# qiaozhijian/VCR-Net

Measured on NVIDIA B200. Metric: pairs/sec @1024 pts, higher is better.
Workload: dtype f16x3-split+f32acc (fp32-equivalent)

## Files before the change

### vcr_net_b200/csrc/knn.cu

```cuda
#include <atomic>
#include "tc_common.cuh"

namespace {

constexpr int TQ = 32;
constexpr int TC = 512;
constexpr int NT = 256;
constexpr int RPL = TC / 32;

template <bool TOKEN_MAJOR>
__global__ void knn_sqnorm_kernel(const float* __restrict__ x, int D, int N, float* __restrict__ xx) {
    const int b = blockIdx.y;
    const int i = blockIdx.x * blockDim.x + threadIdx.x;
    if (i >= N) return;
    const float* xb = x + (size_t)b * D * N;
    float acc = 0.f;
    for (int d = 0; d < D; ++d) {
        const float v = TOKEN_MAJOR ? xb[(size_t)i * D + d] : xb[(size_t)d * N + i];
        acc = fmaf(v, v, acc);
    }
    xx[(size_t)b * N + i] = acc;
}

__device__ __forceinline__ uint32_t okey(float v) {
    const uint32_t b = __float_as_uint(v + 0.f);
    return b ^ (uint32_t)(((int32_t)b >> 31) | 0x80000000);
}
__device__ __forceinline__ float okey_inv(uint32_t k) {
    return __uint_as_float((k & 0x80000000u) ? (k ^ 0x80000000u) : ~k);
}
struct Key { uint32_t hi, lo; };
__device__ __forceinline__ Key key_xchg(Key v, int j, bool take_max) {
    Key o;
    o.hi = __shfl_xor_sync(0xffffffffu, v.hi, j);
    o.lo = __shfl_xor_sync(0xffffffffu, v.lo, j);
    const bool gt = v.hi > o.hi || (v.hi == o.hi && v.lo > o.lo);
    return gt == take_max ? v : o;
}
__device__ __forceinline__ Key key_max(Key a, Key b) {
    return (a.hi > b.hi || (a.hi == b.hi && a.lo > b.lo)) ? a : b;
}

template <int W>
__device__ __forceinline__ void sort32_desc(Key (&v)[W], int lane) {
#pragma unroll
    for (int ks = 2; ks <= 32; ks <<= 1) {
#pragma unroll
        for (int j = ks >> 1; j > 0; j >>= 1) {
            const bool take_max = ((lane & j) == 0) == ((lane & ks) == 0);
#pragma unroll
            for (int w = 0; w < W; ++w) v[w] = key_xchg(v[w], j, take_max);
        }
    }
}
template <int W>
__device__ __forceinline__ void sort32_desc_f(float (&v)[W], int lane) {
#pragma unroll
    for (int ks = 2; ks <= 32; ks <<= 1) {
#pragma unroll
        for (int j = ks >> 1; j > 0; j >>= 1) {
            const bool take_max = ((lane & j) == 0) == ((lane & ks) == 0);
#pragma unroll
            for (int w = 0; w < W; ++w) {
                const float o = __shfl_xor_sync(0xffffffffu, v[w], j);
                v[w] = take_max ? fmaxf(v[w], o) : fminf(v[w], o);
            }
        }
    }
}
template <int W>
__device__ __forceinline__ void merge32_desc(Key (&run)[W], const Key (&add)[W], int lane) {
#pragma unroll
    for (int w = 0; w < W; ++w) {
        Key o;
        o.hi = __shfl_sync(0xffffffffu, add[w].hi, 31 - lane);
        o.lo = __shfl_sync(0xffffffffu, add[w].lo, 31 - lane);
        run[w] = key_max(run[w], o);
    }
#pragma unroll
    for (int j = 16; j > 0; j >>= 1) {
        const bool take_max = (lane & j) == 0;
#pragma unroll
        for (int w = 0; w < W; ++w) run[w] = key_xchg(run[w], j, take_max);
    }
}

template <int W, int TCN, int LDD, int CAP>
__device__ __forceinline__ bool filter_merge_t(const float* drows, const float (&tau)[W], Key (&run)[W], uint2* buf,
                                               int j0, int lane) {
    constexpr int RP = TCN / 32;
    const uint32_t lt = (1u << lane) - 1u;
    int cnt[W], off[W];
    int base = 0;
    __syncwarp();
#pragma unroll
    for (int w = 0; w < W; ++w) {
        const float* dr = drows + w * LDD + lane;
        float v[RP];
#pragma unroll
        for (int r = 0; r < RP; ++r) v[r] = dr[r * 32];
        off[w] = base;
        int n = base;
#pragma unroll
        for (int r = 0; r < RP; ++r) {
            const bool p = v[r] >= tau[w];
            const uint32_t bal = __ballot_sync(0xffffffffu, p);
            const int pos = n + __popc(bal & lt);
            if (p && pos < CAP) buf[pos] = make_uint2(~(uint32_t)(j0 + r * 32 + lane), okey(v[r]));
            n += __popc(bal);
        }
        cnt[w] = n - base;
        base = n;
    }
    __syncwarp();
    if (base > CAP) return false;
    int rounds = 0;
#pragma unroll
    for (int w = 0; w < W; ++w) rounds = max(rounds, (cnt[w] + 31) >> 5);
    for (int r = 0; r < rounds; ++r) {
        Key e[W];
#pragma unroll
        for (int w = 0; w < W; ++w) {
            const int p = r * 32 + lane;
            const uint2 t = p < cnt[w] ? buf[off[w] + p] : make_uint2(0u, 0u);
            e[w].lo = t.x; e[w].hi = t.y;
        }
        sort32_desc<W>(e, lane);
        merge32_desc<W>(run, e, lane);
    }
    return true;
}
template <int W>
__device__ __forceinline__ bool filter_merge(const float* drows, const float (&tau)[W], Key (&run)[W], uint2* buf,
                                             int j0, int lane) {
    return filter_merge_t<W, TC, TC, TC>(drows, tau, run, buf, j0, lane);
}

__device__ __forceinline__ void select_chunk(const float* dist, uint2* surv, Key (&run)[TQ / (NT / 32)], int j0, int kk,
                                             int warp, int lane, bool first) {
    constexpr int QWn = TQ / (NT / 32);
    uint2* buf = surv + (size_t)warp * TC;
    const float* drows = dist + (size_t)(warp * QWn) * TC;
    float tau[QWn];
    if (first) {
        float m[QWn];
#pragma unroll
        for (int w = 0; w < QWn; ++w) {
            const float* dr = drows + w * TC + lane;
            float mm = dr[0];
#pragma unroll
            for (int r = 1; r < RPL; ++r) mm = fmaxf(mm, dr[r * 32]);
            m[w] = mm;
        }
        sort32_desc_f<QWn>(m, lane);
#pragma unroll
        for (int w = 0; w < QWn; ++w) tau[w] = __shfl_sync(0xffffffffu, m[w], kk);
    } else {
#pragma unroll
        for (int w = 0; w < QWn; ++w) tau[w] = okey_inv(__shfl_sync(0xffffffffu, run[w].hi, kk));
    }
    if (!filter_merge<QWn>(drows, tau, run, buf, j0, lane)) {
#pragma unroll
        for (int w = 0; w < QWn; ++w) {
            float t1[1] = {tau[w]};
            Key r1[1] = {run[w]};
            filter_merge<1>(drows + w * TC, t1, r1, buf, j0, lane);
            run[w] = r1[0];
        }
    }
}

__device__ __forceinline__ void cp_async16(float* dst, const float* src, bool valid) {
    const uint32_t d = (uint32_t)__cvta_generic_to_shared(dst);
    const int sz = valid ? 16 : 0;
    asm volatile("cp.async.ca.shared.global [%0], [%1], 16, %2;\n" ::"r"(d), "l"(src), "r"(sz) : "memory");
}
__device__ __forceinline__ void cp_async_wait_all() { asm volatile("cp.async.wait_all;\n" ::: "memory"); }
__device__ __forceinline__ void cp_async_commit() { asm volatile("cp.async.commit_group;\n" ::: "memory"); }
template <int NPEND>
__device__ __forceinline__ void cp_async_wait_group() { asm volatile("cp.async.wait_group %0;\n" ::"n"(NPEND) : "memory"); }

template <int DCH, int DCP>
__device__ __forceinline__ void issue_slab(const float* __restrict__ xb, int D, int N, int j0, int q0, int d0,
                                           float* Cb, float* Qb, int tid) {
    constexpr int PPR = DCH / 4;
    constexpr int RPP = 256 / PPR;
    const int part = tid % PPR, r0 = tid / PPR;
    const bool dok = d0 + 4 * part < D;
    const float* src = xb + (size_t)(j0 + r0) * D + d0 + 4 * part;
    float* dst = Cb + r0 * DCP + 4 * part;
#pragma unroll
    for (int n = 0; n < 512 / RPP; ++n) {
        const bool ok = dok && j0 + r0 + n * RPP < N;
        cp_async16(dst + n * RPP * DCP, ok ? src + (size_t)n * RPP * D : xb, ok);
    }
    if (r0 < 32) {
        const bool ok = dok && q0 + r0 < N;
        cp_async16(Qb + r0 * DCP + 4 * part, ok ? xb + (size_t)(q0 + r0) * D + d0 + 4 * part : xb, ok);
    }
    cp_async_commit();
}

constexpr int QW = TQ / (NT / 32);
constexpr size_t SURV_BYTES = (size_t)(NT / 32) * TC * sizeof(uint2);

template <int DCH>
struct Smem {
    static constexpr int DCP = DCH == 4 ? 12 : DCH + 4;
    static constexpr size_t stage_bytes = (size_t)(TC + TQ) * DCP * sizeof(float);
    static constexpr size_t region0 = stage_bytes > SURV_BYTES ? stage_bytes : SURV_BYTES;
    static constexpr size_t total = region0 + (size_t)TC * sizeof(float) + (size_t)TQ * TC * sizeof(float);
};

template <int DCH, bool TOKEN_MAJOR>
__global__ void __launch_bounds__(NT, 2)
knn_select_kernel(const float* __restrict__ x, const float* __restrict__ xx, int D, int N, int k,
                  int32_t* __restrict__ idx32, int64_t* __restrict__ idx64, const int* __restrict__ redo) {
    if (redo != nullptr && redo[blockIdx.y * gridDim.x + blockIdx.x] == 0) return;
    using S = Smem<DCH>;
    constexpr int DCP = S::DCP;
    extern __shared__ __align__(16) unsigned char smem_raw[];
    float* Cs = reinterpret_cast<float*>(smem_raw);
    float* Qs = Cs + TC * DCP;
    uint2* surv = reinterpret_cast<uint2*>(smem_raw);
    float* xxc = reinterpret_cast<float*>(smem_raw + S::region0);
    float* dist = xxc + TC;

    const int tid = threadIdx.x, lane = tid & 31, warp = tid >> 5;
    const int qg = warp & 3, cg = warp >> 2;
    const int b = blockIdx.y, q0 = blockIdx.x * TQ;
    const float* xb = x + (size_t)b * D * N;
    const float* xxb = xx + (size_t)b * N;
    const bool vec = TOKEN_MAJOR && (D % 4 == 0) && ((reinterpret_cast<uintptr_t>(x) & 15) == 0);

    Key run[QW];
#pragma unroll
    for (int w = 0; w < QW; ++w) run[w].hi = run[w].lo = 0u;

    for (int j0 = 0; j0 < N; j0 += TC) {
        float acc[8][8];
#pragma unroll
        for (int qi = 0; qi < 8; ++qi)
#pragma unroll
            for (int ci = 0; ci < 8; ++ci) acc[qi][ci] = 0.f;

        const int nslab = (D + DCH - 1) / DCH;
        __syncthreads();
        if (vec) issue_slab<DCH, DCP>(xb, D, N, j0, q0, 0, Cs, Qs, tid);
        for (int c = tid; c < TC; c += NT) xxc[c] = (j0 + c < N) ? xxb[j0 + c] : 0.f;
        for (int si = 0; si < nslab; ++si) {
            const int d0 = si * DCH;
            const float* Cb = (vec && (si & 1)) ? dist : Cs;
            const float* Qb = Cb + TC * DCP;
            if (vec) {
                if (si + 1 < nslab) {
                    float* Cn = (si & 1) ? Cs : dist;
                    issue_slab<DCH, DCP>(xb, D, N, j0, q0, d0 + DCH, Cn, Cn + TC * DCP, tid);
                    cp_async_wait_group<1>();
                } else {
                    cp_async_wait_group<0>();
                }
            } else {
                for (int e = tid; e < (TC + TQ) * DCH; e += NT) {
                    int row, d;
                    if (TOKEN_MAJOR) { row = e / DCH; d = e - row * DCH; }
                    else if (e < TC * DCH) { d = e / TC; row = e - d * TC; }
                    else { const int e2 = e - TC * DCH; d = e2 / TQ; row = TC + e2 - d * TQ; }
                    const int g = row < TC ? j0 + row : q0 + (row - TC);
                    float v = 0.f;
                    if (g < N && d0 + d < D)
                        v = TOKEN_MAJOR ? xb[(size_t)g * D + d0 + d] : xb[(size_t)(d0 + d) * N + g];
                    Cs[row * DCP + d] = v;
                }
            }
            __syncthreads();

            const float* qrow = Qb + (qg * 8) * DCP;
            const float* crow = Cb + (cg * 256 + lane) * DCP;
            if (j0 + cg * 256 < N) {
#pragma unroll 1
            for (int d4 = 0; d4 < DCH / 4; ++d4) {
#pragma unroll
                for (int h = 0; h < 2; ++h) {
                    float4 cv[4];
#pragma unroll
                    for (int ci = 0; ci < 4; ++ci)
                        cv[ci] = *reinterpret_cast<const float4*>(crow + ((h * 4 + ci) * 32) * DCP + d4 * 4);
#pragma unroll
                    for (int qi = 0; qi < 8; ++qi) {
                        const float4 qv = *reinterpret_cast<const float4*>(qrow + qi * DCP + d4 * 4);
#pragma unroll
                        for (int ci = 0; ci < 4; ++ci) acc[qi][h * 4 + ci] = fmaf(qv.x, cv[ci].x, acc[qi][h * 4 + ci]);
#pragma unroll
                        for (int ci = 0; ci < 4; ++ci) acc[qi][h * 4 + ci] = fmaf(qv.y, cv[ci].y, acc[qi][h * 4 + ci]);
#pragma unroll
                        for (int ci = 0; ci < 4; ++ci) acc[qi][h * 4 + ci] = fmaf(qv.z, cv[ci].z, acc[qi][h * 4 + ci]);
#pragma unroll
                        for (int ci = 0; ci < 4; ++ci) acc[qi][h * 4 + ci] = fmaf(qv.w, cv[ci].w, acc[qi][h * 4 + ci]);
                    }
                }
            }
            }
            __syncthreads();
        }

        float xxq[8];
#pragma unroll
        for (int qi = 0; qi < 8; ++qi) {
            const int q = q0 + qg * 8 + qi;
            xxq[qi] = q < N ? xxb[q] : 0.f;
        }
#pragma unroll
        for (int ci = 0; ci < 8; ++ci) {
            const int c = cg * 256 + ci * 32 + lane;
            const float nxc = -xxc[c];
            const bool cvalid = j0 + c < N;
#pragma unroll
            for (int qi = 0; qi < 8; ++qi) {
                const float pd = __fsub_rn(__fsub_rn(nxc, -2.f * acc[qi][ci]), xxq[qi]);
                dist[(qg * 8 + qi) * TC + c] = cvalid ? pd : -INFINITY;
            }
        }
        __syncthreads();

        select_chunk(dist, surv, run, j0, k, warp, lane, j0 == 0);
    }

#pragma unroll
    for (int w = 0; w < QW; ++w) {
        const int q = q0 + warp * QW + w;
        if (q < N && lane >= 1 && lane <= k) {
            const int j = (int)(~run[w].lo);
            const size_t o = ((size_t)b * N + q) * k + lane - 1;
            if (idx32) idx32[o] = j;
            if (idx64) idx64[o] = (int64_t)j;
        }
    }
}

template <int DCH, bool TM>
int launch_knn(const float* x, const float* xx, int B, int D, int N, int k, int32_t* i32, int64_t* i64,
               cudaStream_t st, const int* redo = nullptr) {
    auto kern = knn_select_kernel<DCH, TM>;
    const size_t smem = Smem<DCH>::total;
    if (cudaFuncSetAttribute(kern, cudaFuncAttributeMaxDynamicSharedMemorySize, (int)smem) != cudaSuccess) return VCR_ERR_LAUNCH;
    dim3 grid(vcr_cdiv(N, TQ), B);
    kern<<<grid, NT, smem, st>>>(x, xx, D, N, k, i32, i64, redo);
    VCR_CHECK_LAUNCH();
    return VCR_OK;
}

template <int W, class F>
__device__ __forceinline__ bool filter_merge_fn(F&& get, const float (&tau)[W], Key (&run)[W], uint2* buf, int j0, int lane) {
    constexpr int RP = TC / 32;
    const uint32_t lt = (1u << lane) - 1u;
    int cnt[W], off[W];
    int base = 0;
    __syncwarp();
#pragma unroll
    for (int w = 0; w < W; ++w) {
        off[w] = base;
        int n = base;
#pragma unroll
        for (int r = 0; r < RP; ++r) {
            const float v = get(w, r);
            const bool p = v >= tau[w];
            const uint32_t bal = __ballot_sync(0xffffffffu, p);
            const int pos = n + __popc(bal & lt);
            if (p && pos < TC) buf[pos] = make_uint2(~(uint32_t)(j0 + r * 32 + lane), okey(v));
            n += __popc(bal);
        }
        cnt[w] = n - base;
        base = n;
    }
    __syncwarp();
    if (base > TC) return false;
    int rounds = 0;
#pragma unroll
    for (int w = 0; w < W; ++w) rounds = max(rounds, (cnt[w] + 31) >> 5);
    for (int r = 0; r < rounds; ++r) {
        Key e[W];
#pragma unroll
        for (int w = 0; w < W; ++w) {
            const int p = r * 32 + lane;
            const uint2 t = p < cnt[w] ? buf[off[w] + p] : make_uint2(0u, 0u);
            e[w].lo = t.x; e[w].hi = t.y;
        }
        sort32_desc<W>(e, lane);
        merge32_desc<W>(run, e, lane);
    }
    return true;
}

constexpr int QW3 = 2;
constexpr int TQ3 = QW3 * (NT / 32);
template <bool TOKEN_MAJOR>
__global__ void __launch_bounds__(NT, 4)
knn3_kernel(const float* __restrict__ x, const float* __restrict__ xx, int N, int k,
            int32_t* __restrict__ idx32, int64_t* __restrict__ idx64) {
    __shared__ float cs[4][TC];
    __shared__ uint2 surv[NT / 32][TC];
    const int tid = threadIdx.x, lane = tid & 31, warp = tid >> 5;
    const int b = blockIdx.y, q0 = blockIdx.x * TQ3;
    const float* xb = x + (size_t)b * 3 * N;
    const float* xxb = xx + (size_t)b * N;

    float qx[QW3], qy[QW3], qz[QW3], xxq[QW3];
#pragma unroll
    for (int w = 0; w < QW3; ++w) {
        const int q = min(q0 + warp * QW3 + w, N - 1);
        qx[w] = TOKEN_MAJOR ? xb[(size_t)q * 3 + 0] : xb[q];
        qy[w] = TOKEN_MAJOR ? xb[(size_t)q * 3 + 1] : xb[(size_t)N + q];
        qz[w] = TOKEN_MAJOR ? xb[(size_t)q * 3 + 2] : xb[2 * (size_t)N + q];
        xxq[w] = xxb[q];
    }
    Key run[QW3];
#pragma unroll
    for (int w = 0; w < QW3; ++w) run[w].hi = run[w].lo = 0u;
    uint2* buf = surv[warp];

    for (int j0 = 0; j0 < N; j0 += TC) {
        __syncthreads();
        for (int c = tid; c < TC; c += NT) {
            const int g = j0 + c;
            const bool ok = g < N;
            cs[0][c] = ok ? (TOKEN_MAJOR ? xb[(size_t)g * 3 + 0] : xb[g]) : 0.f;
            cs[1][c] = ok ? (TOKEN_MAJOR ? xb[(size_t)g * 3 + 1] : xb[(size_t)N + g]) : 0.f;
            cs[2][c] = ok ? (TOKEN_MAJOR ? xb[(size_t)g * 3 + 2] : xb[2 * (size_t)N + g]) : 0.f;
            cs[3][c] = ok ? xxb[g] : 0.f;
        }
        __syncthreads();
        auto pd = [&](int w, int r) -> float {
            const int c = r * 32 + lane;
            const float acc = fmaf(qz[w], cs[2][c], fmaf(qy[w], cs[1][c], fmaf(qx[w], cs[0][c], 0.f)));
            const float v = __fsub_rn(__fsub_rn(-cs[3][c], -2.f * acc), xxq[w]);
            return j0 + c < N ? v : -INFINITY;
        };
        float tau[QW3];
        if (j0 == 0) {
            float m[QW3];
#pragma unroll
            for (int w = 0; w < QW3; ++w) {
                float mm = pd(w, 0);
#pragma unroll
                for (int r = 1; r < RPL; ++r) mm = fmaxf(mm, pd(w, r));
                m[w] = mm;
            }
            sort32_desc_f<QW3>(m, lane);
#pragma unroll
            for (int w = 0; w < QW3; ++w) tau[w] = __shfl_sync(0xffffffffu, m[w], k);
        } else {
#pragma unroll
            for (int w = 0; w < QW3; ++w) tau[w] = okey_inv(__shfl_sync(0xffffffffu, run[w].hi, k));
        }
        if (!filter_merge_fn<QW3>(pd, tau, run, buf, j0, lane)) {
#pragma unroll
            for (int w = 0; w < QW3; ++w) {
                float t1[1] = {tau[w]};
                Key r1[1] = {run[w]};
                filter_merge_fn<1>([&](int, int r) { return pd(w, r); }, t1, r1, buf, j0, lane);
                run[w] = r1[0];
            }
        }
    }
#pragma unroll
    for (int w = 0; w < QW3; ++w) {
        const int q = q0 + warp * QW3 + w;
        if (q < N && lane >= 1 && lane <= k) {
            const int j = (int)(~run[w].lo);
            const size_t o = ((size_t)b * N + q) * k + lane - 1;
            if (idx32) idx32[o] = j;
            if (idx64) idx64[o] = (int64_t)j;
        }
    }
}

constexpr int T2M = 128;
constexpr int T2TILES = TC / T2M;
constexpr int T2NT = NT + 32;
constexpr int T2CTILE = T2M * 128;
constexpr int T2QTILE = TQ * 128;

struct KnnTcParams {
    const float* x;
    const float* xx;
    const uint32_t* xxmax;
    int* redo;
    int* nflag;
    int D, N, k, ksel, KB;
    int32_t* idx32;
    int64_t* idx64;
};

__host__ __device__ constexpr size_t knn_tc_stage_bytes(int KB) {
    return (size_t)KB * 2 * T2CTILE > SURV_BYTES ? (size_t)KB * 2 * T2CTILE : SURV_BYTES;
}
__host__ __device__ constexpr size_t knn_tc_smem_bytes(int KB) {
    return (size_t)KB * 2 * T2QTILE + knn_tc_stage_bytes(KB) + (size_t)TQ * TC * 4 + TQ * 4 + 64 + 1024;
}

__global__ void knn_sqnorm_max_kernel(const float* __restrict__ x, int D, int N, float* __restrict__ xx,
                                      uint32_t* __restrict__ xxmax) {
    const int b = blockIdx.y;
    const int i = blockIdx.x * blockDim.x + threadIdx.x;
    uint32_t bits = 0u;
    if (i < N) {
        const float* r = x + ((size_t)b * N + i) * D;
        float acc = 0.f;
        for (int d = 0; d < D; ++d) acc = fmaf(r[d], r[d], acc);
        xx[(size_t)b * N + i] = acc;
        bits = __float_as_uint(acc);
    }
    bits = __reduce_max_sync(0xffffffffu, bits);
    if ((threadIdx.x & 31) == 0 && bits) atomicMax(xxmax + b, bits);
}

__global__ void __launch_bounds__(T2NT, 2)
knn_tc_kernel(const __grid_constant__ CUtensorMap tmC, const __grid_constant__ CUtensorMap tmQ, const KnnTcParams p) {
    extern __shared__ uint8_t smem_raw[];
    uint8_t* smem = smem_raw + ((1024u - (tc::smem_u32(smem_raw) & 1023u)) & 1023u);
    const int KB = p.KB, N = p.N, D = p.D, k = p.k, ksel = p.ksel;
    const int qbytes = KB * 2 * T2QTILE, cbytes = KB * 2 * T2CTILE;
    uint8_t* q_s = smem;
    uint8_t* c_s = smem + qbytes;
    uint2* surv = reinterpret_cast<uint2*>(c_s);
    float* dist = reinterpret_cast<float*>(c_s + knn_tc_stage_bytes(KB));
    float* xxq_s = dist + TQ * TC;
    uint64_t* bars = reinterpret_cast<uint64_t*>(xxq_s + TQ);
    uint64_t* q_full = bars + 0;
    uint64_t* c_full = bars + 1;
    uint64_t* mma_bar = bars + 2;
    uint64_t* chunk_ready = bars + 3;
    uint64_t* stage_free = bars + 4;
    uint32_t* tmem_slot = reinterpret_cast<uint32_t*>(bars + 5);

    const int tid = threadIdx.x, warp = tid >> 5, lane = tid & 31;
    const int b = blockIdx.y, q0 = blockIdx.x * TQ;
    const float* xxb = p.xx + (size_t)b * N;
    const int nch = (N + TC - 1) / TC;

    if (warp == NT / 32 && lane == 0) {
        tc::tma_prefetch_desc(&tmC); tc::tma_prefetch_desc(&tmQ);
        tc::mbar_init(q_full, 1); tc::mbar_init(c_full, 1); tc::mbar_init(mma_bar, 1);
        tc::mbar_init(chunk_ready, 1); tc::mbar_init(stage_free, NT / 32);
        tc::fence_barrier_init();
    }
    if (warp == 0) { tc::tmem_alloc(tmem_slot, 256); tc::tmem_relinquish(); }
    if (tid < TQ) xxq_s[tid] = q0 + tid < N ? xxb[q0 + tid] : 0.f;
    tc::tc_fence_before();
    __syncthreads();
    tc::tc_fence_after();
    const uint32_t tmem_base = *tmem_slot;

    const float xm = __uint_as_float(p.xxmax[b]);
    const bool cloud_ok = xm >= 9.5367431640625e-07f && xm <= 1073741824.f;
    if (!cloud_ok) {
        if (tid == 0) {
            p.redo[b * gridDim.x + blockIdx.x] = 1;
            atomicAdd(p.nflag, min(TQ, N - q0));
        }
    } else if (warp == NT / 32) {
        if (tc::elect_one()) {
            constexpr uint32_t idesc = tc::umma_idesc(T2M, TQ, 0);
            const int row0 = b * N;
            tc::mbar_expect_tx(q_full, qbytes);
            for (int kb = 0; kb < KB; ++kb)
                for (int pl = 0; pl < 2; ++pl)
                    tc::tma_load_3d(q_s + (kb * 2 + pl) * T2QTILE, &tmQ, q_full, kb * 64, row0 + q0, pl);
            tc::mbar_wait(q_full, 0);
            const uint32_t q_addr = tc::smem_u32(q_s), c_addr = tc::smem_u32(c_s);
            uint32_t g = 0;
            for (int c = 0; c < nch; ++c) {
                if (c > 0) { tc::mbar_wait(stage_free, (c - 1) & 1); tc::tc_fence_after(); }
                for (int t = 0; t < T2TILES; ++t, ++g) {
                    const int cand0 = c * TC + t * T2M;
                    if (cand0 < N) {
                        tc::mbar_expect_tx(c_full, cbytes);
                        for (int kb = 0; kb < KB; ++kb)
                            for (int pl = 0; pl < 2; ++pl)
                                tc::tma_load_3d(c_s + (kb * 2 + pl) * T2CTILE, &tmC, c_full, kb * 64, row0 + cand0, pl);
                        tc::mbar_wait(c_full, g & 1);
                        tc::tc_fence_after();
                        const uint32_t d0 = tmem_base + t * TQ, d1 = tmem_base + T2TILES * TQ + t * TQ;
                        for (int kb = 0; kb < KB; ++kb) {
                            const uint64_t c_hi = tc::umma_desc_k_sw128(c_addr + (kb * 2) * T2CTILE);
                            const uint64_t c_lo = tc::umma_desc_k_sw128(c_addr + (kb * 2 + 1) * T2CTILE);
                            const uint64_t q_hi = tc::umma_desc_k_sw128(q_addr + (kb * 2) * T2QTILE);
                            const uint64_t q_lo = tc::umma_desc_k_sw128(q_addr + (kb * 2 + 1) * T2QTILE);
#pragma unroll
                            for (int kk = 0; kk < 4; ++kk) {
                                const uint32_t acc = (kb | kk) != 0;
                                const uint64_t adv = (uint64_t)(kk * 2);
                                tc::umma_f16(d0, c_hi + adv, q_hi + adv, idesc, acc);
                                tc::umma_f16(d1, c_hi + adv, q_lo + adv, idesc, acc);
                                tc::umma_f16(d1, c_lo + adv, q_hi + adv, idesc, 1);
                            }
                        }
                        tc::umma_commit(mma_bar);
                        tc::mbar_wait(mma_bar, g & 1);
                    } else {
                        tc::mbar_arrive(c_full);
                        tc::mbar_arrive(mma_bar);
                    }
                }
                tc::umma_commit(chunk_ready);
            }
        }
    } else {
        const int qq = warp & 3, th = warp >> 2;
        Key run[QW];
#pragma unroll
        for (int w = 0; w < QW; ++w) run[w].hi = run[w].lo = 0u;

        for (int c = 0; c < nch; ++c) {
            const int j0 = c * TC;
            tc::mbar_wait(chunk_ready, c & 1);
            tc::tc_fence_after();
#pragma unroll
            for (int tt = 0; tt < T2TILES / 2; ++tt) {
                const int t = th * (T2TILES / 2) + tt;
                const int cl = t * T2M + qq * 32 + lane;
                const int j = j0 + cl;
                float* dcol = dist + cl;
                if (j0 + t * T2M < N) {
                    const uint32_t ta = tmem_base + ((uint32_t)(qq * 32) << 16) + t * TQ;
                    const bool cvalid = j < N;
                    const float nxc = cvalid ? -xxb[j] : 0.f;
#pragma unroll
                    for (int h = 0; h < 2; ++h) {
                        uint32_t r0[16], r1[16];
                        tc::tmem_ld_32x16(ta + h * 16, r0);
                        tc::tmem_ld_32x16(ta + T2TILES * TQ + h * 16, r1);
                        tc::tmem_ld_wait();
#pragma unroll
                        for (int q = 0; q < 16; ++q) {
                            const float dot = fmaf(__uint_as_float(r1[q]), 1.f / 2048.f, __uint_as_float(r0[q]));
                            const float pd = __fsub_rn(__fsub_rn(nxc, -2.f * dot), xxq_s[h * 16 + q]);
                            dcol[(h * 16 + q) * TC] = cvalid ? pd : -INFINITY;
                        }
                    }
                } else {
#pragma unroll
                    for (int q = 0; q < TQ; ++q) dcol[q * TC] = -INFINITY;
                }
            }
            tc::tc_fence_before();
            asm volatile("bar.sync 1, %0;" ::"n"(NT) : "memory");
            select_chunk(dist, surv, run, j0, ksel, warp, lane, c == 0);
            tc::fence_proxy_async();
            __syncwarp();
            if (lane == 0) tc::mbar_arrive(stage_free);
        }

        const bool vec = (D % 4 == 0) && ((reinterpret_cast<uintptr_t>(p.x) & 15) == 0);
        bool all_safe = true;
#pragma unroll
        for (int qi = 0; qi < QW; ++qi) {
            const int q = q0 + warp * QW + qi;
            if (q >= N) continue;
            const Key a = run[qi];
            const uint32_t thr_hi = __shfl_sync(0xffffffffu, a.hi, ksel);
            const int j = (int)(~a.lo);
            const bool valid = j >= 0 && j < N;
            const float xxq = xxq_s[warp * QW + qi];
            Key e[1];
            e[0].hi = 0u; e[0].lo = 0u;
            if (valid) {
                const float* xq = p.x + ((size_t)b * N + q) * D;
                const float* xj = p.x + ((size_t)b * N + j) * D;
                float acc = 0.f;
                if (vec) {
                    for (int d = 0; d < D; d += 4) {
                        const float4 qv = __ldg(reinterpret_cast<const float4*>(xq + d));
                        const float4 cv = __ldg(reinterpret_cast<const float4*>(xj + d));
                        acc = fmaf(qv.x, cv.x, acc); acc = fmaf(qv.y, cv.y, acc);
                        acc = fmaf(qv.z, cv.z, acc); acc = fmaf(qv.w, cv.w, acc);
                    }
                } else {
                    for (int d = 0; d < D; ++d) acc = fmaf(__ldg(xq + d), __ldg(xj + d), acc);
                }
                const float pd = __fsub_rn(__fsub_rn(-xxb[j], -2.f * acc), xxq);
                e[0].hi = okey(pd); e[0].lo = a.lo;
            }
            sort32_desc<1>(e, lane);
            const uint32_t ek_hi = __shfl_sync(0xffffffffu, e[0].hi, k);
            const float eps = 6.103515625e-05f * sqrtf(xxq * xm) + 9.5367431640625e-07f * xm;
            const bool safe = ek_hi != 0u && (thr_hi == 0u || okey_inv(ek_hi) > okey_inv(thr_hi) + eps);
            if (safe) {
                if (lane >= 1 && lane <= k) {
                    const int jn = (int)(~e[0].lo);
                    const size_t o = ((size_t)b * N + q) * k + lane - 1;
                    if (p.idx32) p.idx32[o] = jn;
                    if (p.idx64) p.idx64[o] = (int64_t)jn;
                }
            } else {
                all_safe = false;
                if (lane == 0) atomicAdd(p.nflag, 1);
            }
        }
        if (!all_safe && lane == 0) p.redo[b * gridDim.x + blockIdx.x] = 1;
    }
    tc::tc_fence_before();
    __syncthreads();
    if (warp == 0) tc::tmem_dealloc(tmem_base, 256);
}

#include "knn_tpq.cuh"

}

VCR_API size_t vcr_knn_workspace_bytes(int B, int N) { return (size_t)B * N * sizeof(float); }

static std::atomic<int> g_vcr_knn3_direct{1};
static std::atomic<int> g_vcr_knn_tc_tpq{2};

VCR_API int vcr_set_knn3_direct(int on) {
    return g_vcr_knn3_direct.exchange(on ? 1 : 0);
}

VCR_API int vcr_set_knn_tc_tpq(int on) {
    return g_vcr_knn_tc_tpq.exchange(on < 0 ? 0 : (on > 2 ? 2 : on));
}

VCR_API int vcr_knn_topk(const float* x, int B, int D, int N, int k, int token_major, int32_t* idx32,
                         int64_t* idx64, void* workspace, size_t workspace_bytes, cudaStream_t stream) {
    VCR_REQUIRE(x && (idx32 || idx64) && B > 0 && N > 0 && k >= 1);
    if (N < k + 1) return VCR_ERR_INVALID;
    if (!workspace || workspace_bytes < vcr_knn_workspace_bytes(B, N)) return VCR_ERR_WORKSPACE;
    float* xx = reinterpret_cast<float*>(workspace);
    dim3 g(vcr_cdiv(N, 256), B);
    if (token_major) knn_sqnorm_kernel<true><<<g, 256, 0, stream>>>(x, D, N, xx);
    else knn_sqnorm_kernel<false><<<g, 256, 0, stream>>>(x, D, N, xx);
    VCR_CHECK_LAUNCH();
    if (k > 31) return VCR_ERR_UNSUPPORTED;
    const int route3 = g_vcr_knn3_direct.load(std::memory_order_relaxed);
    if (D == 3 && route3 != 0) {
        dim3 grid(vcr_cdiv(N, TQ3), B);
        if (token_major) knn3_kernel<true><<<grid, NT, 0, stream>>>(x, xx, N, k, idx32, idx64);
        else knn3_kernel<false><<<grid, NT, 0, stream>>>(x, xx, N, k, idx32, idx64);
        VCR_CHECK_LAUNCH();
        return VCR_OK;
    }
    if (D <= 4)
        return token_major ? launch_knn<4, true>(x, xx, B, D, N, k, idx32, idx64, stream)
                           : launch_knn<4, false>(x, xx, B, D, N, k, idx32, idx64, stream);
    return token_major ? launch_knn<16, true>(x, xx, B, D, N, k, idx32, idx64, stream)
                       : launch_knn<16, false>(x, xx, B, D, N, k, idx32, idx64, stream);
}

VCR_API size_t vcr_knn_tc_workspace_bytes(int B, int N) {
    return ((size_t)B * N + (size_t)B + (size_t)B * ((N + 31) / 32) + 1) * 4;
}

VCR_API int vcr_knn_topk_tc(const float* x, const void* xop, int ld, long long plane_stride, int B, int D, int N, int k,
                            int32_t* idx32, int64_t* idx64, void* workspace, size_t workspace_bytes,
                            cudaStream_t stream) {
    VCR_REQUIRE(x && xop && (idx32 || idx64) && B > 0 && N > 0 && k >= 1);
    if (N < k + 1) return VCR_ERR_INVALID;
    if (D < 16 || D > 128 || k > 30 || (long long)B * N > 0x7fffffffLL || B > 65535) return VCR_ERR_UNSUPPORTED;
    if (!workspace || workspace_bytes < vcr_knn_tc_workspace_bytes(B, N)) return VCR_ERR_WORKSPACE;
    const int nq32 = (N + 31) / 32;
    float* xx = reinterpret_cast<float*>(workspace);
    uint32_t* xxmax = reinterpret_cast<uint32_t*>(xx + (size_t)B * N);
    int* redo = reinterpret_cast<int*>(xxmax + B);
    int* nflag = redo + (size_t)B * nq32;
    if (cudaMemsetAsync(xxmax, 0, ((size_t)B + (size_t)B * nq32 + 1) * 4, stream) != cudaSuccess) return VCR_ERR_LAUNCH;
    dim3 g(vcr_cdiv(N, 256), B);
    knn_sqnorm_max_kernel<<<g, 256, 0, stream>>>(x, D, N, xx, xxmax);
    VCR_CHECK_LAUNCH();
    CUtensorMap tmC, tmQ;
    const int tpq = g_vcr_knn_tc_tpq.load(std::memory_order_relaxed);
    if (tpq == 1 || (tpq == 2 && N >= 8192)) {
        int rc = vcr_make_operand_tmap(&tmC, xop, D, (long long)B * N, ld, plane_stride, 2, TC2);
        if (rc != VCR_OK) return rc;
        rc = vcr_make_operand_tmap(&tmQ, xop, D, (long long)B * N, ld, plane_stride, 2, TQ2);
        if (rc != VCR_OK) return rc;
        KnnTcParams p;
        p.x = x; p.xx = xx; p.xxmax = xxmax; p.redo = redo; p.nflag = nflag;
        p.D = D; p.N = N; p.k = k; p.ksel = k + 8 < 31 ? k + 8 : 31; p.KB = (D + 63) / 64;
        p.idx32 = idx32; p.idx64 = idx64;
        const size_t smem = knn_tc2_smem_bytes(p.KB);
        if (cudaFuncSetAttribute(knn_tc2_kernel, cudaFuncAttributeMaxDynamicSharedMemorySize, (int)smem) != cudaSuccess)
            return VCR_ERR_LAUNCH;
        knn_tc2_kernel<<<dim3(vcr_cdiv(N, TQ2), B), T2_THREADS, smem, stream>>>(tmC, tmQ, p);
        VCR_CHECK_LAUNCH();
        return launch_knn<16, true>(x, xx, B, D, N, k, idx32, idx64, stream, redo);
    }
    int rc = vcr_make_operand_tmap(&tmC, xop, D, (long long)B * N, ld, plane_stride, 2, T2M);
    if (rc != VCR_OK) return rc;
    rc = vcr_make_operand_tmap(&tmQ, xop, D, (long long)B * N, ld, plane_stride, 2, TQ);
    if (rc != VCR_OK) return rc;
    KnnTcParams p;
    p.x = x; p.xx = xx; p.xxmax = xxmax; p.redo = redo; p.nflag = nflag;
    p.D = D; p.N = N; p.k = k; p.ksel = k + 8 < 31 ? k + 8 : 31; p.KB = (D + 63) / 64;
    p.idx32 = idx32; p.idx64 = idx64;
    const size_t smem = knn_tc_smem_bytes(p.KB);
    if (cudaFuncSetAttribute(knn_tc_kernel, cudaFuncAttributeMaxDynamicSharedMemorySize, (int)smem) != cudaSuccess)
        return VCR_ERR_LAUNCH;
    knn_tc_kernel<<<dim3(nq32, B), T2NT, smem, stream>>>(tmC, tmQ, p);
    VCR_CHECK_LAUNCH();
    return launch_knn<16, true>(x, xx, B, D, N, k, idx32, idx64, stream, redo);
}
```

Before: 3779.

## Fuse squared norms into kNN kernels, add 384-wide chunks, rewrite filter compaction

For N up to 1024, the separate squared-norm kernel launch is dropped and each select kernel computes candidate and query norms from the staged shared-memory slabs; the D=3 kernel computes them inline. The candidate chunk width becomes a template parameter, and 384 is chosen when it needs no more chunks than 512. The survivor filter now builds per-lane bitmasks and a warp prefix scan instead of one ballot per row, and the first threshold estimate uses two partial maxima per lane. The aim is to cut a launch plus global traffic and reduce padded work and per-row warp ops, at the cost of redundant norm arithmetic and more template instantiations.

```diff
diff --git a/vcr_net_b200/csrc/knn.cu b/vcr_net_b200/csrc/knn.cu
--- a/vcr_net_b200/csrc/knn.cu
+++ b/vcr_net_b200/csrc/knn.cu
@@ -6,7 +6,9 @@
 constexpr int TQ = 32;
 constexpr int TC = 512;
 constexpr int NT = 256;
-constexpr int RPL = TC / 32;
+constexpr int KNN_OWN_NORMS_MAX_N = 1024;
+
+inline int knn_chunk(int N) { return vcr_cdiv(N, 384) <= vcr_cdiv(N, 512) ? 384 : 512; }
 
 template <bool TOKEN_MAJOR>
 __global__ void knn_sqnorm_kernel(const float* __restrict__ x, int D, int N, float* __restrict__ xx) {
@@ -85,35 +87,49 @@
     }
 }
 
-template <int W, int TCN, int LDD, int CAP>
-__device__ __forceinline__ bool filter_merge_t(const float* drows, const float (&tau)[W], Key (&run)[W], uint2* buf,
-                                               int j0, int lane) {
-    constexpr int RP = TCN / 32;
-    const uint32_t lt = (1u << lane) - 1u;
-    int cnt[W], off[W];
+template <int W, int RP, int CAP, class F>
+__device__ __forceinline__ bool filter_merge(F&& get, const float (&tau)[W], Key (&run)[W], uint2* buf, int j0,
+                                             int lane) {
+    static_assert(RP <= 32, "one mask bit per row");
+    uint32_t msk[W];
+    int pre[W], cnt[W], off[W];
+#pragma unroll
+    for (int w = 0; w < W; ++w) {
+        uint32_t m = 0u;
+#pragma unroll
+        for (int r = 0; r < RP; ++r) m |= (uint32_t)(get(w, r) >= tau[w]) << r;
+        msk[w] = m;
+    }
+#pragma unroll
+    for (int w = 0; w < W; ++w) pre[w] = __popc(msk[w]);
+#pragma unroll
+    for (int o = 1; o < 32; o <<= 1) {
+#pragma unroll
+        for (int w = 0; w < W; ++w) {
+            const int t = __shfl_up_sync(0xffffffffu, pre[w], o);
+            if (lane >= o) pre[w] += t;
+        }
+    }
     int base = 0;
+#pragma unroll
+    for (int w = 0; w < W; ++w) {
+        cnt[w] = __shfl_sync(0xffffffffu, pre[w], 31);
+        off[w] = base;
+        base += cnt[w];
+    }
+    if (base > CAP) return false;
     __syncwarp();
 #pragma unroll
     for (int w = 0; w < W; ++w) {
-        const float* dr = drows + w * LDD + lane;
-        float v[RP];
-#pragma unroll
-        for (int r = 0; r < RP; ++r) v[r] = dr[r * 32];
-        off[w] = base;
-        int n = base;
-#pragma unroll
-        for (int r = 0; r < RP; ++r) {
-            const bool p = v[r] >= tau[w];
-            const uint32_t bal = __ballot_sync(0xffffffffu, p);
-            const int pos = n + __popc(bal & lt);
-            if (p && pos < CAP) buf[pos] = make_uint2(~(uint32_t)(j0 + r * 32 + lane), okey(v[r]));
-            n += __popc(bal);
-        }
-        cnt[w] = n - base;
-        base = n;
+        uint32_t m = msk[w];
+        int pos = off[w] + pre[w] - __popc(m);
+        while (m) {
+            const int r = __ffs(m) - 1;
+            m &= m - 1u;
+            buf[pos++] = make_uint2(~(uint32_t)(j0 + r * 32 + lane), okey(get(w, r)));
+        }
     }
     __syncwarp();
-    if (base > CAP) return false;
     int rounds = 0;
 #pragma unroll
     for (int w = 0; w < W; ++w) rounds = max(rounds, (cnt[w] + 31) >> 5);
@@ -130,41 +146,58 @@
     }
     return true;
 }
-template <int W>
-__device__ __forceinline__ bool filter_merge(const float* drows, const float (&tau)[W], Key (&run)[W], uint2* buf,
-                                             int j0, int lane) {
-    return filter_merge_t<W, TC, TC, TC>(drows, tau, run, buf, j0, lane);
-}
-
-__device__ __forceinline__ void select_chunk(const float* dist, uint2* surv, Key (&run)[TQ / (NT / 32)], int j0, int kk,
+
+template <int W, int RP, class F>
+__device__ __forceinline__ void first_tau(F&& get, float (&tau)[W], int nrow, int kk, int lane) {
+    float v[2 * W];
+#pragma unroll
+    for (int w = 0; w < W; ++w) {
+        float h0 = -INFINITY, h1 = -INFINITY;
+#pragma unroll
+        for (int r = 0; r < RP; ++r) {
+            if (r < nrow) {
+                if (r < RP / 2) h0 = fmaxf(h0, get(w, r));
+                else h1 = fmaxf(h1, get(w, r));
+            }
+        }
+        v[w] = h0;
+        v[W + w] = h1;
+    }
+    sort32_desc_f<2 * W>(v, lane);
+#pragma unroll
+    for (int w = 0; w < W; ++w) {
+        float t = fmaxf(v[w], __shfl_sync(0xffffffffu, v[W + w], 31 - lane));
+#pragma unroll
+        for (int j = 16; j > 0; j >>= 1) {
+            const float o = __shfl_xor_sync(0xffffffffu, t, j);
+            t = (lane & j) == 0 ? fmaxf(t, o) : fminf(t, o);
+        }
+        tau[w] = __shfl_sync(0xffffffffu, t, kk);
+    }
+}
+
+constexpr int QW = TQ / (NT / 32);
+
+template <int TCW>
+__device__ __forceinline__ void select_chunk(const float* dist, uint2* surv, Key (&run)[QW], int j0, int nrow, int kk,
                                              int warp, int lane, bool first) {
-    constexpr int QWn = TQ / (NT / 32);
-    uint2* buf = surv + (size_t)warp * TC;
-    const float* drows = dist + (size_t)(warp * QWn) * TC;
-    float tau[QWn];
+    constexpr int RP = TCW / 32;
+    uint2* buf = surv + (size_t)warp * TCW;
+    const float* drows = dist + (size_t)(warp * QW) * TCW + lane;
+    auto get = [&](int w, int r) -> float { return drows[w * TCW + r * 32]; };
+    float tau[QW];
     if (first) {
-        float m[QWn];
-#pragma unroll
-        for (int w = 0; w < QWn; ++w) {
-            const float* dr = drows + w * TC + lane;
-            float mm = dr[0];
-#pragma unroll
-            for (int r = 1; r < RPL; ++r) mm = fmaxf(mm, dr[r * 32]);
-            m[w] = mm;
-        }
-        sort32_desc_f<QWn>(m, lane);
-#pragma unroll
-        for (int w = 0; w < QWn; ++w) tau[w] = __shfl_sync(0xffffffffu, m[w], kk);
+        first_tau<QW, RP>(get, tau, nrow, kk, lane);
     } else {
 #pragma unroll
-        for (int w = 0; w < QWn; ++w) tau[w] = okey_inv(__shfl_sync(0xffffffffu, run[w].hi, kk));
-    }
-    if (!filter_merge<QWn>(drows, tau, run, buf, j0, lane)) {
-#pragma unroll
-        for (int w = 0; w < QWn; ++w) {
+        for (int w = 0; w < QW; ++w) tau[w] = okey_inv(__shfl_sync(0xffffffffu, run[w].hi, kk));
+    }
+    if (!filter_merge<QW, RP, TCW>(get, tau, run, buf, j0, lane)) {
+#pragma unroll
+        for (int w = 0; w < QW; ++w) {
             float t1[1] = {tau[w]};
             Key r1[1] = {run[w]};
-            filter_merge<1>(drows + w * TC, t1, r1, buf, j0, lane);
+            filter_merge<1, RP, TCW>([&](int, int r) { return get(w, r); }, t1, r1, buf, j0, lane);
             run[w] = r1[0];
         }
     }
@@ -180,93 +213,109 @@
 template <int NPEND>
 __device__ __forceinline__ void cp_async_wait_group() { asm volatile("cp.async.wait_group %0;\n" ::"n"(NPEND) : "memory"); }
 
-template <int DCH, int DCP>
+template <int DCH, int DCP, int TCW>
 __device__ __forceinline__ void issue_slab(const float* __restrict__ xb, int D, int N, int j0, int q0, int d0,
                                            float* Cb, float* Qb, int tid) {
     constexpr int PPR = DCH / 4;
-    constexpr int RPP = 256 / PPR;
+    constexpr int RPP = NT / PPR;
     const int part = tid % PPR, r0 = tid / PPR;
     const bool dok = d0 + 4 * part < D;
     const float* src = xb + (size_t)(j0 + r0) * D + d0 + 4 * part;
     float* dst = Cb + r0 * DCP + 4 * part;
 #pragma unroll
-    for (int n = 0; n < 512 / RPP; ++n) {
-        const bool ok = dok && j0 + r0 + n * RPP < N;
-        cp_async16(dst + n * RPP * DCP, ok ? src + (size_t)n * RPP * D : xb, ok);
-    }
-    if (r0 < 32) {
+    for (int n = 0; n < (TCW + RPP - 1) / RPP; ++n) {
+        if (TCW % RPP == 0 || r0 + n * RPP < TCW) {
+            const bool ok = dok && j0 + r0 + n * RPP < N;
+            cp_async16(dst + n * RPP * DCP, ok ? src + (size_t)n * RPP * D : xb, ok);
+        }
+    }
+    if (r0 < TQ) {
         const bool ok = dok && q0 + r0 < N;
         cp_async16(Qb + r0 * DCP + 4 * part, ok ? xb + (size_t)(q0 + r0) * D + d0 + 4 * part : xb, ok);
     }
     cp_async_commit();
 }
 
-constexpr int QW = TQ / (NT / 32);
 constexpr size_t SURV_BYTES = (size_t)(NT / 32) * TC * sizeof(uint2);
 
-template <int DCH>
+template <int DCH, int TCW>
 struct Smem {
     static constexpr int DCP = DCH == 4 ? 12 : DCH + 4;
-    static constexpr size_t stage_bytes = (size_t)(TC + TQ) * DCP * sizeof(float);
-    static constexpr size_t region0 = stage_bytes > SURV_BYTES ? stage_bytes : SURV_BYTES;
-    static constexpr size_t total = region0 + (size_t)TC * sizeof(float) + (size_t)TQ * TC * sizeof(float);
+    static constexpr size_t stage_bytes = (size_t)(TCW + TQ) * DCP * sizeof(float);
+    static constexpr size_t surv_bytes = (size_t)(NT / 32) * TCW * sizeof(uint2);
+    static constexpr size_t region0 = stage_bytes > surv_bytes ? stage_bytes : surv_bytes;
+    static constexpr size_t dist_bytes = (size_t)TQ * TCW * sizeof(float);
+    static constexpr size_t total = region0 + (size_t)(TCW + TQ) * sizeof(float) + dist_bytes;
+    static_assert(stage_bytes <= dist_bytes, "the second operand buffer aliases the distance tile");
 };
 
-template <int DCH, bool TOKEN_MAJOR>
+template <int DCH, bool TOKEN_MAJOR, int TCW>
 __global__ void __launch_bounds__(NT, 2)
 knn_select_kernel(const float* __restrict__ x, const float* __restrict__ xx, int D, int N, int k,
                   int32_t* __restrict__ idx32, int64_t* __restrict__ idx64, const int* __restrict__ redo) {
     if (redo != nullptr && redo[blockIdx.y * gridDim.x + blockIdx.x] == 0) return;
-    using S = Smem<DCH>;
+    using S = Smem<DCH, TCW>;
     constexpr int DCP = S::DCP;
+    constexpr int HC = TCW / 2;
+    constexpr int CH = TCW / 128;
+    constexpr int NH = TCW == 384 ? 1 : 2, CPH = 2 * CH / NH;
+    constexpr int RP = TCW / 32;
+    constexpr int NR = (TCW + NT - 1) / NT;
     extern __shared__ __align__(16) unsigned char smem_raw[];
     float* Cs = reinterpret_cast<float*>(smem_raw);
-    float* Qs = Cs + TC * DCP;
+    float* Qs = Cs + TCW * DCP;
     uint2* surv = reinterpret_cast<uint2*>(smem_raw);
     float* xxc = reinterpret_cast<float*>(smem_raw + S::region0);
-    float* dist = xxc + TC;
+    float* xxq_s = xxc + TCW;
+    float* dist = xxq_s + TQ;
 
     const int tid = threadIdx.x, lane = tid & 31, warp = tid >> 5;
     const int qg = warp & 3, cg = warp >> 2;
     const int b = blockIdx.y, q0 = blockIdx.x * TQ;
     const float* xb = x + (size_t)b * D * N;
-    const float* xxb = xx + (size_t)b * N;
+    const bool own_xx = xx == nullptr;
+    const float* xxb = own_xx ? nullptr : xx + (size_t)b * N;
     const bool vec = TOKEN_MAJOR && (D % 4 == 0) && ((reinterpret_cast<uintptr_t>(x) & 15) == 0);
 
     Key run[QW];
 #pragma unroll
     for (int w = 0; w < QW; ++w) run[w].hi = run[w].lo = 0u;
 
-    for (int j0 = 0; j0 < N; j0 += TC) {
-        float acc[8][8];
+    const int nch = (N + TCW - 1) / TCW, c0 = own_xx ? q0 / TCW : 0;
+    for (int cc = 0; cc < nch; ++cc) {
+        const int j0 = (c0 + cc < nch ? c0 + cc : c0 + cc - nch) * TCW;
+        float acc[8][2 * CH];
 #pragma unroll
         for (int qi = 0; qi < 8; ++qi)
 #pragma unroll
-            for (int ci = 0; ci < 8; ++ci) acc[qi][ci] = 0.f;
+            for (int ci = 0; ci < 2 * CH; ++ci) acc[qi][ci] = 0.f;
 
         const int nslab = (D + DCH - 1) / DCH;
         __syncthreads();
-        if (vec) issue_slab<DCH, DCP>(xb, D, N, j0, q0, 0, Cs, Qs, tid);
-        for (int c = tid; c < TC; c += NT) xxc[c] = (j0 + c < N) ? xxb[j0 + c] : 0.f;
+        if (vec) issue_slab<DCH, DCP, TCW>(xb, D, N, j0, q0, 0, Cs, Qs, tid);
+        if (!own_xx) {
+            for (int c = tid; c < TCW; c += NT) xxc[c] = (j0 + c < N) ? xxb[j0 + c] : 0.f;
+            if (tid < TQ) xxq_s[tid] = q0 + tid < N ? xxb[q0 + tid] : 0.f;
+        }
         for (int si = 0; si < nslab; ++si) {
             const int d0 = si * DCH;
             const float* Cb = (vec && (si & 1)) ? dist : Cs;
-            const float* Qb = Cb + TC * DCP;
+            const float* Qb = Cb + TCW * DCP;
             if (vec) {
                 if (si + 1 < nslab) {
                     float* Cn = (si & 1) ? Cs : dist;
-                    issue_slab<DCH, DCP>(xb, D, N, j0, q0, d0 + DCH, Cn, Cn + TC * DCP, tid);
+                    issue_slab<DCH, DCP, TCW>(xb, D, N, j0, q0, d0 + DCH, Cn, Cn + TCW * DCP, tid);
                     cp_async_wait_group<1>();
                 } else {
                     cp_async_wait_group<0>();
                 }
             } else {
-                for (int e = tid; e < (TC + TQ) * DCH; e += NT) {
+                for (int e = tid; e < (TCW + TQ) * DCH; e += NT) {
                     int row, d;
                     if (TOKEN_MAJOR) { row = e / DCH; d = e - row * DCH; }
-                    else if (e < TC * DCH) { d = e / TC; row = e - d * TC; }
-                    else { const int e2 = e - TC * DCH; d = e2 / TQ; row = TC + e2 - d * TQ; }
-                    const int g = row < TC ? j0 + row : q0 + (row - TC);
+                    else if (e < TCW * DCH) { d = e / TCW; row = e - d * TCW; }
+                    else { const int e2 = e - TCW * DCH; d = e2 / TQ; row = TCW + e2 - d * TQ; }
+                    const int g = row < TCW ? j0 + row : q0 + (row - TCW);
                     float v = 0.f;
                     if (g < N && d0 + d < D)
                         v = TOKEN_MAJOR ? xb[(size_t)g * D + d0 + d] : xb[(size_t)(d0 + d) * N + g];
@@ -276,54 +325,69 @@
             __syncthreads();
 
             const float* qrow = Qb + (qg * 8) * DCP;
-            const float* crow = Cb + (cg * 256 + lane) * DCP;
-            if (j0 + cg * 256 < N) {
+            const float* crow = Cb + (cg * HC + lane) * DCP;
+            if (j0 + cg * HC < N) {
 #pragma unroll 1
             for (int d4 = 0; d4 < DCH / 4; ++d4) {
 #pragma unroll
-                for (int h = 0; h < 2; ++h) {
-                    float4 cv[4];
-#pragma unroll
-                    for (int ci = 0; ci < 4; ++ci)
-                        cv[ci] = *reinterpret_cast<const float4*>(crow + ((h * 4 + ci) * 32) * DCP + d4 * 4);
+                for (int h = 0; h < NH; ++h) {
+                    float4 cv[CPH];
+#pragma unroll
+                    for (int ci = 0; ci < CPH; ++ci)
+                        cv[ci] = *reinterpret_cast<const float4*>(crow + ((h * CPH + ci) * 32) * DCP + d4 * 4);
 #pragma unroll
                     for (int qi = 0; qi < 8; ++qi) {
                         const float4 qv = *reinterpret_cast<const float4*>(qrow + qi * DCP + d4 * 4);
 #pragma unroll
-                        for (int ci = 0; ci < 4; ++ci) acc[qi][h * 4 + ci] = fmaf(qv.x, cv[ci].x, acc[qi][h * 4 + ci]);
-#pragma unroll
-                        for (int ci = 0; ci < 4; ++ci) acc[qi][h * 4 + ci] = fmaf(qv.y, cv[ci].y, acc[qi][h * 4 + ci]);
-#pragma unroll
-                        for (int ci = 0; ci < 4; ++ci) acc[qi][h * 4 + ci] = fmaf(qv.z, cv[ci].z, acc[qi][h * 4 + ci]);
-#pragma unroll
-                        for (int ci = 0; ci < 4; ++ci) acc[qi][h * 4 + ci] = fmaf(qv.w, cv[ci].w, acc[qi][h * 4 + ci]);
+                        for (int ci = 0; ci < CPH; ++ci) acc[qi][h * CPH + ci] = fmaf(qv.x, cv[ci].x, acc[qi][h * CPH + ci]);
+#pragma unroll
+                        for (int ci = 0; ci < CPH; ++ci) acc[qi][h * CPH + ci] = fmaf(qv.y, cv[ci].y, acc[qi][h * CPH + ci]);
+#pragma unroll
+                        for (int ci = 0; ci < CPH; ++ci) acc[qi][h * CPH + ci] = fmaf(qv.z, cv[ci].z, acc[qi][h * CPH + ci]);
+#pragma unroll
+                        for (int ci = 0; ci < CPH; ++ci) acc[qi][h * CPH + ci] = fmaf(qv.w, cv[ci].w, acc[qi][h * CPH + ci]);
                     }
                 }
             }
             }
+            if (own_xx) {
+#pragma unroll
+                for (int i = 0; i < NR; ++i) {
+                    const int r = tid + i * NT;
+                    if (TCW % NT == 0 || r < TCW) {
+                        float a = si == 0 ? 0.f : xxc[r];
+#pragma unroll
+                        for (int d4 = 0; d4 < DCH / 4; ++d4) {
+                            const float4 v = *reinterpret_cast<const float4*>(Cb + r * DCP + d4 * 4);
+                            a = fmaf(v.x, v.x, a); a = fmaf(v.y, v.y, a);
+                            a = fmaf(v.z, v.z, a); a = fmaf(v.w, v.w, a);
+                        }
+                        xxc[r] = a;
+                        const int qr = j0 + r - q0;
+                        if (si == nslab - 1 && (unsigned)qr < (unsigned)TQ) xxq_s[qr] = a;
+                    }
+                }
+            }
             __syncthreads();
         }
 
         float xxq[8];
 #pragma unroll
-        for (int qi = 0; qi < 8; ++qi) {
-            const int q = q0 + qg * 8 + qi;
-            xxq[qi] = q < N ? xxb[q] : 0.f;
-        }
-#pragma unroll
-        for (int ci = 0; ci < 8; ++ci) {
-            const int c = cg * 256 + ci * 32 + lane;
+        for (int qi = 0; qi < 8; ++qi) xxq[qi] = xxq_s[qg * 8 + qi];
+#pragma unroll
+        for (int ci = 0; ci < 2 * CH; ++ci) {
+            const int c = cg * HC + ci * 32 + lane;
             const float nxc = -xxc[c];
             const bool cvalid = j0 + c < N;
 #pragma unroll
             for (int qi = 0; qi < 8; ++qi) {
                 const float pd = __fsub_rn(__fsub_rn(nxc, -2.f * acc[qi][ci]), xxq[qi]);
-                dist[(qg * 8 + qi) * TC + c] = cvalid ? pd : -INFINITY;
+                dist[(qg * 8 + qi) * TCW + c] = cvalid ? pd : -INFINITY;
             }
         }
         __syncthreads();
 
-        select_chunk(dist, surv, run, j0, k, warp, lane, j0 == 0);
+        select_chunk<TCW>(dist, surv, run, j0, min(RP, (N - j0 + 31) >> 5), k, warp, lane, cc == 0);
     }
 
 #pragma unroll
@@ -338,72 +402,35 @@
     }
 }
 
-template <int DCH, bool TM>
-int launch_knn(const float* x, const float* xx, int B, int D, int N, int k, int32_t* i32, int64_t* i64,
-               cudaStream_t st, const int* redo = nullptr) {
-    auto kern = knn_select_kernel<DCH, TM>;
-    const size_t smem = Smem<DCH>::total;
+template <int DCH, bool TM, int TCW>
+int launch_knn_w(const float* x, const float* xx, int B, int D, int N, int k, int32_t* i32, int64_t* i64,
+                 cudaStream_t st, const int* redo) {
+    auto kern = knn_select_kernel<DCH, TM, TCW>;
+    const size_t smem = Smem<DCH, TCW>::total;
     if (cudaFuncSetAttribute(kern, cudaFuncAttributeMaxDynamicSharedMemorySize, (int)smem) != cudaSuccess) return VCR_ERR_LAUNCH;
     dim3 grid(vcr_cdiv(N, TQ), B);
     kern<<<grid, NT, smem, st>>>(x, xx, D, N, k, i32, i64, redo);
     VCR_CHECK_LAUNCH();
     return VCR_OK;
 }
-
-template <int W, class F>
-__device__ __forceinline__ bool filter_merge_fn(F&& get, const float (&tau)[W], Key (&run)[W], uint2* buf, int j0, int lane) {
-    constexpr int RP = TC / 32;
-    const uint32_t lt = (1u << lane) - 1u;
-    int cnt[W], off[W];
-    int base = 0;
-    __syncwarp();
-#pragma unroll
-    for (int w = 0; w < W; ++w) {
-        off[w] = base;
-        int n = base;
-#pragma unroll
-        for (int r = 0; r < RP; ++r) {
-            const float v = get(w, r);
-            const bool p = v >= tau[w];
-            const uint32_t bal = __ballot_sync(0xffffffffu, p);
-            const int pos = n + __popc(bal & lt);
-            if (p && pos < TC) buf[pos] = make_uint2(~(uint32_t)(j0 + r * 32 + lane), okey(v));
-            n += __popc(bal);
-        }
-        cnt[w] = n - base;
-        base = n;
-    }
-    __syncwarp();
-    if (base > TC) return false;
-    int rounds = 0;
-#pragma unroll
-    for (int w = 0; w < W; ++w) rounds = max(rounds, (cnt[w] + 31) >> 5);
-    for (int r = 0; r < rounds; ++r) {
-        Key e[W];
-#pragma unroll
-        for (int w = 0; w < W; ++w) {
-            const int p = r * 32 + lane;
-            const uint2 t = p < cnt[w] ? buf[off[w] + p] : make_uint2(0u, 0u);
-            e[w].lo = t.x; e[w].hi = t.y;
-        }
-        sort32_desc<W>(e, lane);
-        merge32_desc<W>(run, e, lane);
-    }
-    return true;
+template <int DCH, bool TM>
+int launch_knn(const float* x, const float* xx, int B, int D, int N, int k, int32_t* i32, int64_t* i64,
+               cudaStream_t st, const int* redo = nullptr) {
+    return knn_chunk(N) == 384 ? launch_knn_w<DCH, TM, 384>(x, xx, B, D, N, k, i32, i64, st, redo)
+                               : launch_knn_w<DCH, TM, 512>(x, xx, B, D, N, k, i32, i64, st, redo);
 }
 
 constexpr int QW3 = 2;
 constexpr int TQ3 = QW3 * (NT / 32);
-template <bool TOKEN_MAJOR>
+template <bool TOKEN_MAJOR, int TCW>
 __global__ void __launch_bounds__(NT, 4)
-knn3_kernel(const float* __restrict__ x, const float* __restrict__ xx, int N, int k,
-            int32_t* __restrict__ idx32, int64_t* __restrict__ idx64) {
-    __shared__ float cs[4][TC];
-    __shared__ uint2 surv[NT / 32][TC];
+knn3_kernel(const float* __restrict__ x, int N, int k, int32_t* __restrict__ idx32, int64_t* __restrict__ idx64) {
+    constexpr int RP = TCW / 32;
+    __shared__ float cs[4][TCW];
+    __shared__ uint2 surv[NT / 32][TCW];
     const int tid = threadIdx.x, lane = tid & 31, warp = tid >> 5;
     const int b = blockIdx.y, q0 = blockIdx.x * TQ3;
     const float* xb = x + (size_t)b * 3 * N;
-    const float* xxb = xx + (size_t)b * N;
 
     float qx[QW3], qy[QW3], qz[QW3], xxq[QW3];
 #pragma unroll
@@ -412,22 +439,25 @@
         qx[w] = TOKEN_MAJOR ? xb[(size_t)q * 3 + 0] : xb[q];
         qy[w] = TOKEN_MAJOR ? xb[(size_t)q * 3 + 1] : xb[(size_t)N + q];
         qz[w] = TOKEN_MAJOR ? xb[(size_t)q * 3 + 2] : xb[2 * (size_t)N + q];
-        xxq[w] = xxb[q];
+        xxq[w] = fmaf(qz[w], qz[w], fmaf(qy[w], qy[w], fmaf(qx[w], qx[w], 0.f)));
     }
     Key run[QW3];
 #pragma unroll
     for (int w = 0; w < QW3; ++w) run[w].hi = run[w].lo = 0u;
     uint2* buf = surv[warp];
 
-    for (int j0 = 0; j0 < N; j0 += TC) {
+    for (int j0 = 0; j0 < N; j0 += TCW) {
         __syncthreads();
-        for (int c = tid; c < TC; c += NT) {
+        for (int c = tid; c < TCW; c += NT) {
             const int g = j0 + c;
             const bool ok = g < N;
-            cs[0][c] = ok ? (TOKEN_MAJOR ? xb[(size_t)g * 3 + 0] : xb[g]) : 0.f;
-            cs[1][c] = ok ? (TOKEN_MAJOR ? xb[(size_t)g * 3 + 1] : xb[(size_t)N + g]) : 0.f;
-            cs[2][c] = ok ? (TOKEN_MAJOR ? xb[(size_t)g * 3 + 2] : xb[2 * (size_t)N + g]) : 0.f;
-            cs[3][c] = ok ? xxb[g] : 0.f;
+            const float cx = ok ? (TOKEN_MAJOR ? xb[(size_t)g * 3 + 0] : xb[g]) : 0.f;
+            const float cy = ok ? (TOKEN_MAJOR ? xb[(size_t)g * 3 + 1] : xb[(size_t)N + g]) : 0.f;
+            const float cz = ok ? (TOKEN_MAJOR ? xb[(size_t)g * 3 + 2] : xb[2 * (size_t)N + g]) : 0.f;
+            cs[0][c] = cx;
+            cs[1][c] = cy;
+            cs[2][c] = cz;
+            cs[3][c] = fmaf(cz, cz, fmaf(cy, cy, fmaf(cx, cx, 0.f)));
         }
         __syncthreads();
         auto pd = [&](int w, int r) -> float {
@@ -436,29 +466,20 @@
             const float v = __fsub_rn(__fsub_rn(-cs[3][c], -2.f * acc), xxq[w]);
             return j0 + c < N ? v : -INFINITY;
         };
+        const int nrow = min(RP, (N - j0 + 31) >> 5);
         float tau[QW3];
         if (j0 == 0) {
-            float m[QW3];
-#pragma unroll
-            for (int w = 0; w < QW3; ++w) {
-                float mm = pd(w, 0);
-#pragma unroll
-                for (int r = 1; r < RPL; ++r) mm = fmaxf(mm, pd(w, r));
-                m[w] = mm;
-            }
-            sort32_desc_f<QW3>(m, lane);
-#pragma unroll
-            for (int w = 0; w < QW3; ++w) tau[w] = __shfl_sync(0xffffffffu, m[w], k);
+            first_tau<QW3, RP>(pd, tau, nrow, k, lane);
         } else {
 #pragma unroll
             for (int w = 0; w < QW3; ++w) tau[w] = okey_inv(__shfl_sync(0xffffffffu, run[w].hi, k));
         }
-        if (!filter_merge_fn<QW3>(pd, tau, run, buf, j0, lane)) {
+        if (!filter_merge<QW3, RP, TCW>(pd, tau, run, buf, j0, lane)) {
 #pragma unroll
             for (int w = 0; w < QW3; ++w) {
                 float t1[1] = {tau[w]};
                 Key r1[1] = {run[w]};
-                filter_merge_fn<1>([&](int, int r) { return pd(w, r); }, t1, r1, buf, j0, lane);
+                filter_merge<1, RP, TCW>([&](int, int r) { return pd(w, r); }, t1, r1, buf, j0, lane);
                 run[w] = r1[0];
             }
         }
@@ -473,6 +494,12 @@
             if (idx64) idx64[o] = (int64_t)j;
         }
     }
+}
+template <bool TM>
+void launch_knn3(const float* x, int B, int N, int k, int32_t* i32, int64_t* i64, cudaStream_t st) {
+    const dim3 grid(vcr_cdiv(N, TQ3), B);
+    if (knn_chunk(N) == 384) knn3_kernel<TM, 384><<<grid, NT, 0, st>>>(x, N, k, i32, i64);
+    else knn3_kernel<TM, 512><<<grid, NT, 0, st>>>(x, N, k, i32, i64);
 }
 
 constexpr int T2M = 128;
@@ -646,7 +673,7 @@
             }
             tc::tc_fence_before();
             asm volatile("bar.sync 1, %0;" ::"n"(NT) : "memory");
-            select_chunk(dist, surv, run, j0, ksel, warp, lane, c == 0);
+            select_chunk<TC>(dist, surv, run, j0, min(TC / 32, (N - j0 + 31) >> 5), ksel, warp, lane, c == 0);
             tc::fence_proxy_async();
             __syncwarp();
             if (lane == 0) tc::mbar_arrive(stage_free);
@@ -727,19 +754,21 @@
     VCR_REQUIRE(x && (idx32 || idx64) && B > 0 && N > 0 && k >= 1);
     if (N < k + 1) return VCR_ERR_INVALID;
     if (!workspace || workspace_bytes < vcr_knn_workspace_bytes(B, N)) return VCR_ERR_WORKSPACE;
-    float* xx = reinterpret_cast<float*>(workspace);
-    dim3 g(vcr_cdiv(N, 256), B);
-    if (token_major) knn_sqnorm_kernel<true><<<g, 256, 0, stream>>>(x, D, N, xx);
-    else knn_sqnorm_kernel<false><<<g, 256, 0, stream>>>(x, D, N, xx);
-    VCR_CHECK_LAUNCH();
     if (k > 31) return VCR_ERR_UNSUPPORTED;
     const int route3 = g_vcr_knn3_direct.load(std::memory_order_relaxed);
     if (D == 3 && route3 != 0) {
-        dim3 grid(vcr_cdiv(N, TQ3), B);
-        if (token_major) knn3_kernel<true><<<grid, NT, 0, stream>>>(x, xx, N, k, idx32, idx64);
-        else knn3_kernel<false><<<grid, NT, 0, stream>>>(x, xx, N, k, idx32, idx64);
+        if (token_major) launch_knn3<true>(x, B, N, k, idx32, idx64, stream);
+        else launch_knn3<false>(x, B, N, k, idx32, idx64, stream);
         VCR_CHECK_LAUNCH();
         return VCR_OK;
+    }
+    float* xx = nullptr;
+    if (N > KNN_OWN_NORMS_MAX_N) {
+        xx = reinterpret_cast<float*>(workspace);
+        dim3 g(vcr_cdiv(N, 256), B);
+        if (token_major) knn_sqnorm_kernel<true><<<g, 256, 0, stream>>>(x, D, N, xx);
+        else knn_sqnorm_kernel<false><<<g, 256, 0, stream>>>(x, D, N, xx);
+        VCR_CHECK_LAUNCH();
     }
     if (D <= 4)
         return token_major ? launch_knn<4, true>(x, xx, B, D, N, k, idx32, idx64, stream)
```

Result: no change. 3802 (median of 6 runs) (+0.6%).
